# tensorboy/centerpose

Measured on AMD Instinct MI355X. Metric: images/sec end-to-end (backbone+decode), DLA-34 512x512, higher is better.
Workload: dtype f32

## Files before the change

### centerpose_amd/csrc/head_wino24.hip

```cpp
#include "igemm.h"

#define HW_THREADS 512
#define HW_PH 18
#define HW_PW 18
#define HW_PWP 20
#define HW_C 64
#define HW_CGS (HW_C / 4)
#define HW_CG (HW_PH * HW_PWP * 4)
#define HW_PATCH (HW_CGS * HW_CG)
#define HW_F4 (HW_PH * HW_PW * HW_CGS)
#define HW_SLOTS ((HW_F4 + HW_THREADS - 1) / HW_THREADS)
#define HW_LDR 36
#define HW_RED (16 * 32 * HW_LDR)
#define HW_LDM 36
#define HW_MID (256 * HW_LDM)
#define HW_SMEM_FLOATS (2 * HW_RED)
#define HW_SMEM_FLOATS_MM (HW_RED + HW_MID > HW_PATCH ? HW_RED + HW_MID : HW_PATCH)

typedef float hw_v2 __attribute__((ext_vector_type(2)));
typedef float hw_v4 __attribute__((ext_vector_type(4)));

struct HwHead {
    const float* w2;
    const float* b2;
    float* out2;
    int n2, ld2, act2;
};
struct HwGrid {
    int tilesX, tilesY;
    unsigned mTx, mTy;
};
__device__ __forceinline__ hw_v4 hw_lds4(const float* p) { return *reinterpret_cast<const hw_v4*>(p); }
__device__ __forceinline__ int hw_div(int n, int d, unsigned magic) { return d == 1 ? n : (int)__umulhi((unsigned)n, magic); }

template <int N2, int MM>
__global__ __launch_bounds__(HW_THREADS, 1) void head_wino24_kernel(const ConvArgs a, const HwGrid gd, const HwHead hd)
{
    extern __shared__ __attribute__((aligned(16))) float smem[];
    const int tid = threadIdx.x, lane = tid & 63, wv = __builtin_amdgcn_readfirstlane(tid >> 6);
    const int xi = wv & 3, vh = wv >> 2;
    const int h = lane >> 5, m = lane & 31;
    const int NTILES = (a.Cout + 31) >> 5;
    int t_ = ig_xcd_remap(blockIdx.x, gridDim.x), q_;
    q_ = hw_div(t_, gd.tilesX, gd.mTx); const int tx = t_ - q_ * gd.tilesX; t_ = q_;
    q_ = hw_div(t_, gd.tilesY, gd.mTy); const int ty = t_ - q_ * gd.tilesY;
    const int b = q_;
    const int y0 = ty * 16, x0 = tx * 16;
    const int ld = a.srcLd[0];
    const float* __restrict__ x = a.src[0];

    {
        float4 rg[HW_SLOTS];
        int lo[HW_SLOTS];
        bool ok[HW_SLOTS];
#pragma unroll
        for (int s = 0; s < HW_SLOTS; ++s) {
            const int idx = tid + s * HW_THREADS;
            const int pp = idx / HW_CGS, q = idx % HW_CGS;
            const int py = pp / HW_PW, px = pp - py * HW_PW;
            const int gy = y0 - 1 + py, gx = x0 - 1 + px;
            const bool inl = idx < HW_F4;
            ok[s] = inl && gy >= 0 && gy < a.H && gx >= 0 && gx < a.W;
            const int go = ok[s] ? ((b * a.H + gy) * a.W + gx) * ld + q * 4 : 0;
            lo[s] = inl ? ((q * HW_PH + py) * HW_PWP + (px ^ ((py >> 1) & 3))) * 4 : -1;
            rg[s] = ig_ldg4(x + go);
        }
#pragma unroll
        for (int s = 0; s < HW_SLOTS; ++s)
            if (lo[s] >= 0) {
                float4 v = rg[s];
                if (!ok[s]) v = make_float4(0.f, 0.f, 0.f, 0.f);
                *reinterpret_cast<float4*>(smem + lo[s]) = v;
            }
    }
    const float* up = a.w + ((size_t)xi * NTILES * (HW_C / 8)) * 1536 + (size_t)(3 * vh) * 256 + lane * 4;
    const int nlin = NTILES * (HW_C / 8);
    float4 bq[2][3];
#pragma unroll
    for (int nu = 0; nu < 3; ++nu) bq[0][nu] = ig_ldg4(up + nu * 256);
    __syncthreads();

    const int rA = xi == 0 ? 0 : (xi == 2 ? 2 : 1);
    const int rB = xi == 2 ? 1 : (xi == 3 ? 3 : 2);
    const float sg1 = xi == 1 ? 1.f : -1.f;
    const hw_v2 sg = {sg1, sg1};
    const int tyy = m >> 2, txx = m & 3;
    const int sA = (tyy + (rA >> 1)) & 3, sB = (tyy + (rB >> 1)) & 3;
    const int baseA = ((2 * tyy + rA) * HW_PWP + 4 * txx) * 4 + h * HW_CG;
    const int baseB = ((2 * tyy + rB) * HW_PWP + 4 * txx) * 4 + h * HW_CG;
    int offA[4], offB[4];
#pragma unroll
    for (int jj = 0; jj < 4; ++jj) { offA[jj] = baseA + ((jj ^ sA) << 2); offB[jj] = baseB + ((jj ^ sB) << 2); }
    hw_v2 vl[HW_C / 8][3], vhh[HW_C / 8][3];
#pragma unroll
    for (int kc = 0; kc < HW_C / 8; ++kc) {
        const float* pc = smem + kc * 2 * HW_CG;
        hw_v2 tl[5], th[5];
        if (vh == 0) {
#pragma unroll
            for (int j = 0; j < 5; ++j) {
                const hw_v4 da = hw_lds4(pc + offA[j & 3] + (j >> 2) * 16), db = hw_lds4(pc + offB[j & 3] + (j >> 2) * 16);
                tl[j] = __builtin_elementwise_fma(sg, db.xy, da.xy);
                th[j] = __builtin_elementwise_fma(sg, db.zw, da.zw);
            }
        } else {
#pragma unroll
            for (int j = 0; j < 5; ++j) {
                const int jc = j + 1;
                const hw_v4 da = hw_lds4(pc + offA[jc & 3] + (jc >> 2) * 16), db = hw_lds4(pc + offB[jc & 3] + (jc >> 2) * 16);
                tl[j] = __builtin_elementwise_fma(sg, db.xy, da.xy);
                th[j] = __builtin_elementwise_fma(sg, db.zw, da.zw);
            }
        }
        const hw_v2 k4 = {4.f, 4.f}, kn4 = {-4.f, -4.f}, k2 = {2.f, 2.f}, kn2 = {-2.f, -2.f};
        if (vh == 0) {
            const hw_v2 al = __builtin_elementwise_fma(kn4, tl[2], tl[4]), ah = __builtin_elementwise_fma(kn4, th[2], th[4]);
            const hw_v2 bl = __builtin_elementwise_fma(kn4, tl[1], tl[3]), bh = __builtin_elementwise_fma(kn4, th[1], th[3]);
            vl[kc][0] = __builtin_elementwise_fma(k4, tl[0] - tl[2], tl[4] - tl[2]); vhh[kc][0] = __builtin_elementwise_fma(k4, th[0] - th[2], th[4] - th[2]);
            vl[kc][1] = al + bl; vhh[kc][1] = ah + bh;
            vl[kc][2] = al - bl; vhh[kc][2] = ah - bh;
        } else {
            const hw_v2 cl = tl[3] - tl[1], ch = th[3] - th[1];
            const hw_v2 fl = tl[2] - tl[0], fh = th[2] - th[0];
            vl[kc][0] = __builtin_elementwise_fma(k2, fl, cl); vhh[kc][0] = __builtin_elementwise_fma(k2, fh, ch);
            vl[kc][1] = __builtin_elementwise_fma(kn2, fl, cl); vhh[kc][1] = __builtin_elementwise_fma(kn2, fh, ch);
            vl[kc][2] = __builtin_elementwise_fma(kn4, fl, tl[4] - tl[2]); vhh[kc][2] = __builtin_elementwise_fma(kn4, fh, th[4] - th[2]);
        }
#pragma unroll
        for (int nu = 0; nu < 3; ++nu) asm volatile("" : "+v"(vl[kc][nu]), "+v"(vhh[kc][nu]));
        __builtin_amdgcn_sched_barrier(0);
    }
    __syncthreads();

    float acc2[2][2][N2 > 0 ? N2 : 1];
#pragma unroll
    for (int i = 0; i < 2; ++i)
#pragma unroll
        for (int k = 0; k < 2; ++k)
#pragma unroll
            for (int j = 0; j < (N2 > 0 ? N2 : 1); ++j) acc2[i][k][j] = 0.f;
    f32x16 acc2m;
#pragma unroll
    for (int r = 0; r < 16; ++r) acc2m[r] = 0.f;
    constexpr int J0 = MM ? 32 : 0;
    float* const mid = smem + HW_RED;
    const int n4 = tid & 7, bb = (tid >> 3) & 1, mi = tid >> 4;
    const int ity = mi >> 2, itx = mi & 3;
    const int itrd = (bb * 32 + mi) * HW_LDR + n4 * 4;
    const int wpo = (wv * 64 + m) * HW_LDR + 4 * h;

    int lin = 0;
    if constexpr (!MM) {
        hw_v4 sc = {0.f, 0.f, 0.f, 0.f}, sh = sc, w2r[N2];
#pragma unroll
        for (int j = 0; j < N2; ++j) w2r[j] = sc;
        hw_v4 rq[8];
        auto red_read = [&](int P) __attribute__((always_inline)) {
            int rbase = itrd + P * HW_RED;
            asm volatile("" : "+v"(rbase));
            const float* rp = smem + rbase;
#pragma unroll
            for (int w = 0; w < 8; ++w) rq[w] = hw_lds4(rp + w * 64 * HW_LDR);
        };
        auto red_sum = [&](int P) __attribute__((always_inline)) {
            const hw_v4 r0 = rq[0] + rq[4], r1 = rq[1] + rq[5], r2 = rq[2] + rq[6], r3 = rq[3] + rq[7];
            hw_v4 yv[2];
            yv[0] = (r0 + r1) + r2;
            yv[1] = (r1 - r2) - r3;
#pragma unroll
            for (int aa = 0; aa < 2; ++aa) {
                hw_v4 v = __builtin_elementwise_fma(yv[aa], sc, sh);
                v = (hw_v4){cp_relu(v.x), cp_relu(v.y), cp_relu(v.z), cp_relu(v.w)};
#pragma unroll
                for (int j = 0; j < N2; ++j) {
                    const hw_v4 w = w2r[j];
                    acc2[P][aa][j] = fmaf(v.w, w.w, fmaf(v.z, w.z, fmaf(v.y, w.y, fmaf(v.x, w.x, acc2[P][aa][j]))));
                }
            }
        };
#pragma unroll 1
        for (int nt = 0; nt < NTILES; ++nt) {
            const bool prev = nt > 0;
            f32x16 acc[3];
#pragma unroll
            for (int nu = 0; nu < 3; ++nu)
#pragma unroll
                for (int r = 0; r < 16; ++r) acc[nu][r] = 0.f;
#pragma unroll
            for (int kc = 0; kc < HW_C / 8; ++kc) {
                ++lin;
                const float* un = up + (size_t)(lin < nlin ? lin : nlin - 1) * 1536;
                __builtin_amdgcn_sched_barrier(0);
#pragma unroll
                for (int nu = 0; nu < 3; ++nu) {
                    if (nu == 1) {
#pragma unroll
                        for (int q = 0; q < 3; ++q) bq[(kc + 1) & 1][q] = ig_ldg4(un + q * 256);
                        __builtin_amdgcn_sched_barrier(0);
                    }
                    if (nu == 2 && prev) {
                        if (kc == 0) red_read(0);
                        if (kc == 2) red_sum(0);
                        if (kc == 4) red_read(1);
                        if (kc == 6) red_sum(1);
                        __builtin_amdgcn_sched_barrier(0);
                    }
                    const float4 bbv = bq[kc & 1][nu];
                    acc[nu] = __builtin_amdgcn_mfma_f32_32x32x2f32(bbv.x, vl[kc][nu].x, acc[nu], 0, 0, 0);
                    acc[nu] = __builtin_amdgcn_mfma_f32_32x32x2f32(bbv.y, vl[kc][nu].y, acc[nu], 0, 0, 0);
                    acc[nu] = __builtin_amdgcn_mfma_f32_32x32x2f32(bbv.z, vhh[kc][nu].x, acc[nu], 0, 0, 0);
                    acc[nu] = __builtin_amdgcn_mfma_f32_32x32x2f32(bbv.w, vhh[kc][nu].y, acc[nu], 0, 0, 0);
                }
                __builtin_amdgcn_sched_barrier(0);
            }
            const int ncol = nt * 32 + n4 * 4;
            sc = *reinterpret_cast<const hw_v4*>(a.scale + ncol);
            sh = *reinterpret_cast<const hw_v4*>(a.shift + ncol);
#pragma unroll
            for (int j = 0; j < N2; ++j) w2r[j] = *reinterpret_cast<const hw_v4*>(hd.w2 + (size_t)j * hd.ld2 + ncol);
            if (prev) __syncthreads();
#pragma unroll
            for (int P = 0; P < 2; ++P) {
                int wbase = wpo + P * HW_RED;
                asm volatile("" : "+v"(wbase));
                float* wq = smem + wbase;
#pragma unroll
                for (int j = 0; j < 4; ++j) {
                    hw_v4 q[3];
#pragma unroll
                    for (int nu = 0; nu < 3; ++nu) q[nu] = (hw_v4){acc[nu][4 * j], acc[nu][4 * j + 1], acc[nu][4 * j + 2], acc[nu][4 * j + 3]};
                    hw_v4 c0, c1;
                    if (vh == 0) {
                        const hw_v4 s1 = q[1] + q[2], d1 = q[1] - q[2];
                        c0 = P == 0 ? q[0] + s1 : s1;
                        c1 = d1;
                    } else {
                        const hw_v4 s2 = q[0] + q[1], d2 = q[0] - q[1];
                        c0 = P == 0 ? s2 : 4.f * s2;
                        c1 = P == 0 ? 2.f * d2 : 8.f * d2 + q[2];
                    }
                    *reinterpret_cast<hw_v4*>(wq + 8 * j) = c0;
                    *reinterpret_cast<hw_v4*>(wq + 32 * HW_LDR + 8 * j) = c1;
                }
            }
            __syncthreads();
        }
        red_read(0); red_sum(0);
        red_read(1); red_sum(1);
    } else {
#pragma unroll 1
    for (int nt = 0; nt < NTILES; ++nt) {
        f32x16 acc[3];
#pragma unroll
        for (int nu = 0; nu < 3; ++nu)
#pragma unroll
            for (int r = 0; r < 16; ++r) acc[nu][r] = 0.f;
#pragma unroll
        for (int kc = 0; kc < HW_C / 8; ++kc) {
            ++lin;
            const float* un = up + (size_t)(lin < nlin ? lin : nlin - 1) * 1536;
            __builtin_amdgcn_sched_barrier(0);
#pragma unroll
            for (int nu = 0; nu < 3; ++nu) {
                if (nu == 1) {
#pragma unroll
                    for (int q = 0; q < 3; ++q) bq[(kc + 1) & 1][q] = ig_ldg4(un + q * 256);
                    __builtin_amdgcn_sched_barrier(0);
                }
                const float4 bbv = bq[kc & 1][nu];
                acc[nu] = __builtin_amdgcn_mfma_f32_32x32x2f32(bbv.x, vl[kc][nu].x, acc[nu], 0, 0, 0);
                acc[nu] = __builtin_amdgcn_mfma_f32_32x32x2f32(bbv.y, vl[kc][nu].y, acc[nu], 0, 0, 0);
                acc[nu] = __builtin_amdgcn_mfma_f32_32x32x2f32(bbv.z, vhh[kc][nu].x, acc[nu], 0, 0, 0);
                acc[nu] = __builtin_amdgcn_mfma_f32_32x32x2f32(bbv.w, vhh[kc][nu].y, acc[nu], 0, 0, 0);
            }
            __builtin_amdgcn_sched_barrier(0);
        }

        const int ncol = nt * 32 + n4 * 4;
        const hw_v4 sc = *reinterpret_cast<const hw_v4*>(a.scale + ncol), sh = *reinterpret_cast<const hw_v4*>(a.shift + ncol);
        hw_v4 w2r[N2 > 0 ? N2 : 1];
#pragma unroll
        for (int j = 0; j < N2; ++j) w2r[j] = *reinterpret_cast<const hw_v4*>(hd.w2 + (size_t)(J0 + j) * hd.ld2 + ncol);
        hw_v4 w2f[MM ? 4 : 1];
#pragma unroll
        for (int P = 0; P < 2; ++P) {
            if (MM && P == 1) __syncthreads();
            int wbase = wpo + (MM ? 0 : P * HW_RED), rbase = itrd + (MM ? 0 : P * HW_RED);
            asm volatile("" : "+v"(wbase), "+v"(rbase));
            float* wq = smem + wbase;
#pragma unroll
            for (int j = 0; j < 4; ++j) {
                hw_v4 q[3];
#pragma unroll
                for (int nu = 0; nu < 3; ++nu) q[nu] = (hw_v4){acc[nu][4 * j], acc[nu][4 * j + 1], acc[nu][4 * j + 2], acc[nu][4 * j + 3]};
                hw_v4 c0, c1;
                if (vh == 0) {
                    const hw_v4 s1 = q[1] + q[2], d1 = q[1] - q[2];
                    c0 = P == 0 ? q[0] + s1 : s1;
                    c1 = d1;
                } else {
                    const hw_v4 s2 = q[0] + q[1], d2 = q[0] - q[1];
                    c0 = P == 0 ? s2 : 4.f * s2;
                    c1 = P == 0 ? 2.f * d2 : 8.f * d2 + q[2];
                }
                *reinterpret_cast<hw_v4*>(wq + 8 * j) = c0;
                *reinterpret_cast<hw_v4*>(wq + 32 * HW_LDR + 8 * j) = c1;
            }
            if constexpr (MM) {
                if (P == 1) {
                    const int nmm = hd.n2 < 32 ? hd.n2 : 32;
                    const bool live = m < nmm;
                    const float* wrow = hd.w2 + (size_t)(live ? m : nmm - 1) * hd.ld2 + nt * 32 + 4 * h;
#pragma unroll
                    for (int s4 = 0; s4 < 4; ++s4) {
                        const float4 t4 = ig_ldg4(wrow + 8 * s4);
                        w2f[s4] = live ? (hw_v4){t4.x, t4.y, t4.z, t4.w} : (hw_v4){0.f, 0.f, 0.f, 0.f};
                    }
                }
            }
            __syncthreads();
            const float* rp = smem + rbase;
            hw_v4 r0 = hw_lds4(rp) + hw_lds4(rp + 4 * 64 * HW_LDR);
            const hw_v4 r1 = hw_lds4(rp + 64 * HW_LDR) + hw_lds4(rp + 5 * 64 * HW_LDR);
            const hw_v4 r2 = hw_lds4(rp + 2 * 64 * HW_LDR) + hw_lds4(rp + 6 * 64 * HW_LDR);
            const hw_v4 r3 = hw_lds4(rp + 3 * 64 * HW_LDR) + hw_lds4(rp + 7 * 64 * HW_LDR);
            hw_v4 yv[2];
            yv[0] = (r0 + r1) + r2;
            yv[1] = (r1 - r2) - r3;
#pragma unroll
            for (int aa = 0; aa < 2; ++aa) {
                hw_v4 v = __builtin_elementwise_fma(yv[aa], sc, sh);
                v = (hw_v4){cp_relu(v.x), cp_relu(v.y), cp_relu(v.z), cp_relu(v.w)};
#pragma unroll
                for (int j = 0; j < N2; ++j) {
                    const hw_v4 w = w2r[j];
                    acc2[P][aa][j] = fmaf(v.w, w.w, fmaf(v.z, w.z, fmaf(v.y, w.y, fmaf(v.x, w.x, acc2[P][aa][j]))));
                }
                if constexpr (MM) {
                    *reinterpret_cast<hw_v4*>(mid + ((2 * ity + aa) * 16 + 4 * itx + 2 * P + bb) * HW_LDM + n4 * 4) = v;
                }
            }
        }
        if constexpr (MM) {
            __syncthreads();
            const float* mp = mid + (32 * wv + m) * HW_LDM + 4 * h;
            hw_v4 mf[4];
#pragma unroll
            for (int s4 = 0; s4 < 4; ++s4) mf[s4] = hw_lds4(mp + 8 * s4);
#pragma unroll
            for (int s4 = 0; s4 < 4; ++s4) {
                acc2m = __builtin_amdgcn_mfma_f32_32x32x2f32(w2f[s4].x, mf[s4].x, acc2m, 0, 0, 0);
                acc2m = __builtin_amdgcn_mfma_f32_32x32x2f32(w2f[s4].y, mf[s4].y, acc2m, 0, 0, 0);
                acc2m = __builtin_amdgcn_mfma_f32_32x32x2f32(w2f[s4].z, mf[s4].z, acc2m, 0, 0, 0);
                acc2m = __builtin_amdgcn_mfma_f32_32x32x2f32(w2f[s4].w, mf[s4].w, acc2m, 0, 0, 0);
            }
            __syncthreads();
        }
    }

    }
    const size_t HW = (size_t)a.H * a.W;
    if constexpr (MM) {
        const int p = 32 * wv + m, ox = x0 + (p & 15), oy = y0 + (p >> 4);
        const int nmm = hd.n2 < 32 ? hd.n2 : 32;
        if (ox < a.W && oy < a.H) {
#pragma unroll
            for (int r = 0; r < 16; ++r) {
                const int j = (r & 3) + 8 * (r >> 2) + 4 * h;
                if (j < nmm) hd.out2[((size_t)b * hd.n2 + j) * HW + (size_t)oy * a.W + ox] = cp_act(acc2m[r] + hd.b2[j], hd.act2);
            }
        }
    }
    if constexpr (N2 > 0) {
#pragma unroll
        for (int P = 0; P < 2; ++P) {
            const int ox = x0 + 4 * itx + 2 * P + bb, oy = y0 + 2 * ity;
#pragma unroll
            for (int aa = 0; aa < 2; ++aa)
#pragma unroll
                for (int j = 0; j < N2; ++j) {
                    float v = acc2[P][aa][j];
                    v += __shfl_xor(v, 1);
                    v += __shfl_xor(v, 2);
                    v += __shfl_xor(v, 4);
                    if ((tid & 7) == 0 && J0 + j < hd.n2 && ox < a.W && oy + aa < a.H)
                        hd.out2[((size_t)b * hd.n2 + J0 + j) * HW + (size_t)(oy + aa) * a.W + ox] = cp_act(v + hd.b2[J0 + j], hd.act2);
                }
        }
    }
}

static unsigned hw_magic(int d) { return d <= 1 ? 0u : (unsigned)(((1ull << 32) + (unsigned)d - 1) / (unsigned)d); }

template <int N2, int MM>
static int launch_head_wino24(const ConvArgs& a, hipStream_t s, const HwHead& hd)
{
    const int smem = (MM ? HW_SMEM_FLOATS_MM : HW_SMEM_FLOATS) * 4;
    static CpLdsGuard guard;
    {
        const hipError_t e = guard.ensure((const void*)head_wino24_kernel<N2, MM>, smem);
        if (e != hipSuccess) { cp_set_error("head_wino24: cannot reserve %d B LDS: %s", smem, hipGetErrorString(e)); return 2; }
    }
    HwGrid gd;
    gd.tilesX = cp_cdiv(a.W, 16); gd.tilesY = cp_cdiv(a.H, 16);
    gd.mTx = hw_magic(gd.tilesX); gd.mTy = hw_magic(gd.tilesY);
    const long long grid = (long long)a.B * gd.tilesX * gd.tilesY;
    const long long dmax = gd.tilesX > gd.tilesY ? gd.tilesX : gd.tilesY;
    if (grid * dmax >= (1ll << 32)) { cp_set_error("head_wino24: grid %lld too large", grid); return 1; }
    hipLaunchKernelGGL((head_wino24_kernel<N2, MM>), dim3((unsigned)grid), dim3(HW_THREADS), smem, s, a, gd, hd);
    cp_note_kernel("head_wino24_kernel<%d, %d>", N2, MM);
    return 0;
}

int cp_launch_head3x3_1x1_w24(const ConvArgs& a, const float* w2, const float* b2, float* out2, int n2, int ld2, int act2, hipStream_t s)
{
    const bool ok = a.nsrc == 1 && a.kh == 3 && a.kw == 3 && a.sy == 1 && a.sx == 1 && a.py == 1 && a.px == 1 && a.Ho == a.H &&
                    a.Wo == a.W && a.srcC[0] == 64 && a.srcLd[0] % 4 == 0 && a.Cout % 32 == 0 && a.act == CP_ACT_RELU && !a.res &&
                    n2 >= 1 && n2 <= 34 && ld2 % 4 == 0 && ld2 >= a.Cout &&
                    (((size_t)a.src[0] | (size_t)a.w | (size_t)w2 | (size_t)a.scale | (size_t)a.shift) & 15) == 0 &&
                    (long long)a.B * a.H * a.W * a.srcLd[0] < (1ll << 31);
    if (!ok) return -1;
    HwHead hd;
    hd.w2 = w2; hd.b2 = b2; hd.out2 = out2; hd.n2 = n2; hd.ld2 = ld2; hd.act2 = act2;
    if (n2 == 1) return launch_head_wino24<1, 0>(a, s, hd);
    if (n2 == 2) return launch_head_wino24<2, 0>(a, s, hd);
    if (n2 <= 32) return launch_head_wino24<0, 1>(a, s, hd);
    if (n2 == 33) return launch_head_wino24<1, 1>(a, s, hd);
    return launch_head_wino24<2, 1>(a, s, hd);
}
```

### centerpose_amd/ops.py

```python
import ctypes
import os

import torch

from . import _lib

ACT_NONE, ACT_RELU, ACT_SIGMOID, ACT_HSWISH, ACT_HSIGMOID = 0, 1, 2, 3, 4
BN_EPS = 1e-5


class ConvDesc(ctypes.Structure):
    _fields_ = [(n, ctypes.c_int) for n in ("nsrc",)] + [("srcC", ctypes.c_int * 4), ("srcLd", ctypes.c_int * 4)] + \
        [(n, ctypes.c_int) for n in ("B", "H", "W", "Ho", "Wo", "kh", "kw", "sy", "sx", "py", "px", "K", "ldw", "Cout",
                                     "resLd", "outLd", "outNCHW", "OH", "OW", "osy", "osx", "ooy", "oox", "act",
                                     "inNCHW", "tile", "nsub", "ksplit")]


class DcnDesc(ctypes.Structure):
    _fields_ = [(n, ctypes.c_int) for n in ("B", "H", "W", "C", "srcLd", "Ho", "Wo", "kh", "kw", "sy", "sx", "py", "px",
                                            "dily", "dilx", "K", "ldw", "Cout", "omLd", "omSigmoid", "outLd",
                                            "outNCHW", "act", "tile", "ksplit", "dg")]


def round_up(x, m):
# ... 150 lines not shown
        t.stride(0) == t.shape[1] * t.stride(1), "NHWC tensor with dense pixels expected"
    return t.stride(2)


BATCH_INVARIANT = os.environ.get("CP_BATCH_INVARIANT", "0") == "1"


def rule_batch(B):
    return 1 if BATCH_INVARIANT else B


SPLIT_BF16 = os.environ.get("CP_SPLIT_BF16", "0") == "1"
SPLIT_BF16_TILES = ((128, 128), (128, 64), (64, 128), (64, 64))


def split_bf16_weight(wp, ldw):
    L = _lib.lib()
    rows, K = wp.shape
    assert rows % ldw == 0 and K % 16 == 0 and wp.is_contiguous()
    L.cp_split_bf16_weight_floats.restype = ctypes.c_size_t
    wb = torch.empty((L.cp_split_bf16_weight_floats(rows, K),), dtype=torch.float32, device=wp.device)
    _lib.check(L.cp_split_bf16_weights_f32(_lib.ptr(wp), rows, ldw, K, _lib.ptr(wb), _lib.stream()), "cp_split_bf16_weights_f32")
    return wb


def split_bf16_tile(M, ldw, nsub=1, ksplit=1, force=False, K=None):
    if ldw % 64:
        return None
    code = lambda bm, bn: 3000000 + bm * 1000 + bn
    forced = os.environ.get("CP_SPLIT_BF16_TILE")
    if forced:
        bm, bn = (int(v) for v in forced.split("x")) if "x" in forced else (128, int(forced))
        return code(bm, bn if ldw % bn == 0 else 64)
    blocks = lambda bm, bn: ((M + bm - 1) // bm) * max(1, nsub) * max(1, ksplit) * (ldw // bn)
    floor = 0 if force else int(os.environ.get("CP_SPLIT_BF16_MINBLOCKS", "512"))
    if floor == 0:
        return code(128, 128) if ldw % 128 == 0 and blocks(128, 128) >= 256 else code(128, 64)
    if ksplit > 1:
        return None
    order = ((64, 64),) if K is not None and K <= 64 else ((128, 128), (64, 128), (64, 64))
    for bm, bn in order:
        if ldw % bn == 0 and blocks(bm, bn) >= floor:
            return code(bm, bn)
    return None


def conv2d(srcs, wp, scale, shift, out, **kw):
    conv2d_launch(srcs, wp, scale, shift, out, **kw).run()
    return out


def conv2d_launch(srcs, wp, scale, shift, out, *, kh, kw, stride=1, pad=0, cout, act=ACT_NONE, res=None, out_nchw=False,
                  in_nchw=False, Ho=None, Wo=None, pad_yx=None, out_scatter=None, tile=0, wino=None, nsub=1, ksplit=0, split_bf16=None):
    d = ConvDesc()
    d.nsrc = len(srcs)
    if in_nchw:
        x = srcs[0]
        B, C, H, W = x.shape
        d.srcC[0], d.srcLd[0] = C, 0
        assert x.is_contiguous()
    else:
        B, H, W, _ = srcs[0].shape
        for i, s in enumerate(srcs):
            assert s.shape[:3] == srcs[0].shape[:3]
            d.srcC[i], d.srcLd[i] = s.shape[3], _ld(s)
    py, px = pad_yx if pad_yx is not None else (pad, pad)
    if Ho is None:
        Ho = (H + 2 * py - kh) // stride + 1
        Wo = (W + 2 * px - kw) // stride + 1
    d.B, d.H, d.W, d.Ho, d.Wo = B, H, W, Ho, Wo
    d.kh, d.kw, d.sy, d.sx, d.py, d.px = kh, kw, stride, stride, py, px
    assert wp.shape[0] % nsub == 0
    d.K, d.ldw, d.Cout, d.nsub = wp.shape[1], wp.shape[0] // nsub, cout, nsub
    d.resLd = _ld(res) if res is not None else 0
    d.outNCHW = 1 if out_nchw else 0
    d.ksplit = ksplit
    if ksplit > 1:
        assert res is None and act == ACT_NONE and not out_nchw and out.is_contiguous() and (wino is not None or (len(srcs) == 1 and not in_nchw and nsub == 1))
        assert tuple(out.shape[:2]) == (ksplit, B * Ho * Wo) and out.shape[2] >= cout and out.shape[2] % 4 == 0
        d.OH, d.OW, d.outLd = Ho, Wo, out.shape[2]
    elif out_nchw:
        d.OH, d.OW, d.outLd = out.shape[2], out.shape[3], 0
        assert out.is_contiguous() and out.shape[1] == cout
    else:
        d.OH, d.OW, d.outLd = out.shape[1], out.shape[2], _ld(out)
    d.osy, d.osx, d.ooy, d.oox = out_scatter if out_scatter is not None else (1, 1, 0, 0)
    d.act, d.inNCHW, d.tile = act, 1 if in_nchw else 0, tile
    for t in (wp, scale, shift, wino):
        assert t is None or t.is_contiguous()
    if wino is not None:
        assert len(srcs) == 1 and not in_nchw
        return Launch("cp_conv3x3_winograd_f32", d, [srcs[0], wino, scale, shift, res, out])
    if (SPLIT_BF16 if split_bf16 is None else split_bf16) and tile == 0 and not in_nchw:
        code = split_bf16_tile(rule_batch(B) * Ho * Wo, d.ldw, nsub, ksplit, force=split_bf16 is True, K=d.K)
        c16 = kh == 3 and kw == 3 and len(srcs) == 1 and srcs[0].shape[3] == 16 and cout <= 32
        if code is not None and not c16 and all(s.data_ptr() % 16 == 0 for s in srcs):
            d.tile = code
            wp = split_bf16_weight(wp, d.ldw)
    return Launch("cp_conv2d_f32", d, list(srcs) + [None] * (4 - len(srcs)) + [wp, scale, shift, res, out])


ConvDesc4 = ConvDesc * 4


def conv3x3_group_launch(members, whole):
    assert 1 <= len(members) <= 4
    members = sorted(members, key=lambda mm: -mm["x"].shape[3])
    d = ConvDesc4()
    cols = [[None] * 4 for _ in range(6)]
    for i, mm in enumerate(members):
        one = conv2d_launch([mm["x"]], mm["wp"], mm["scale"], mm["shift"], mm["out"], kh=3, kw=3, stride=1, pad=1, cout=mm["cout"],
                            act=mm["act"], res=mm["res"], wino=mm["u24"], tile=WINO24)
        ctypes.memmove(ctypes.addressof(d[i]), ctypes.addressof(one.desc), ctypes.sizeof(ConvDesc))
        for k, t in enumerate((mm["x"], mm["u24"], mm["scale"], mm["shift"], mm["res"], mm["out"])):
            cols[k][i] = t
            assert t is None or k in (0, 4, 5) or t.is_contiguous()
        assert mm["out"].untyped_storage().data_ptr() == whole.untyped_storage().data_ptr()
    return Launch("cp_conv3x3_winograd24_group_f32", d, [t for col in cols for t in col] + [whole], [len(members)])


ConvDesc8 = ConvDesc * 8
GROUP_MAX = 8


def conv2d_group_launch(members, whole):
    assert 1 <= len(members) <= GROUP_MAX
    members = sorted(members, key=lambda mm: -mm["wp"].shape[1])
    d = ConvDesc8()
    cols = [[None] * GROUP_MAX for _ in range(6)]
    for i, mm in enumerate(members):
        assert mm["wp"].shape[0] % 64 == 0
        one = conv2d_launch([mm["x"]], mm["wp"], mm["scale"], mm["shift"], mm["out"], kh=mm["k"], kw=mm["k"], stride=mm["stride"],
                            pad=mm["pad"], cout=mm["cout"], act=mm["act"], res=mm.get("res"), split_bf16=False)
        ctypes.memmove(ctypes.addressof(d[i]), ctypes.addressof(one.desc), ctypes.sizeof(ConvDesc))
        for k, t in enumerate((mm["x"], mm["wp"], mm["scale"], mm["shift"], mm.get("res"), mm["out"])):
            cols[k][i] = t
            assert t is None or k in (0, 4, 5) or t.is_contiguous()
        assert mm["out"].untyped_storage().data_ptr() == whole.untyped_storage().data_ptr()
    return Launch("cp_conv2d_group_f32", d, [t for col in cols for t in col] + [whole], [len(members)])


def head3x3_1x1_eligible(x, hc, n2):
    B, H, W, C = x.shape
    B = rule_batch(B)
    return C == 64 and hc % 32 == 0 and hc >= 128 and 1 <= n2 <= 34 and B * ((H + 7) // 8) * ((W + 15) // 16) >= 512


def head_wino24_wanted(x, n2):
    B, H, W, _ = x.shape
    B = rule_batch(B)
    mode = os.environ.get("CP_HEAD24", "1")
    if mode == "0" or B * ((H + 15) // 16) * ((W + 15) // 16) < 256:
        return False
    return mode == "all" or n2 <= 32


def head3x3_1x1_launch(x, u, scale, shift, w2, b2, out2, *, hc, act2=ACT_NONE, wino24=False):
    B, H, W, C = x.shape
    n2, ld2 = w2.shape
    assert out2.is_contiguous() and tuple(out2.shape) == (B, n2, H, W) and w2.is_contiguous() and b2.numel() >= n2
    d = ConvDesc()
    d.nsrc = 1
    d.srcC[0], d.srcLd[0] = C, _ld(x)
    d.B, d.H, d.W, d.Ho, d.Wo = B, H, W, H, W
    d.kh, d.kw, d.sy, d.sx, d.py, d.px = 3, 3, 1, 1, 1, 1
    d.K, d.ldw, d.Cout = 9 * C, round_up(hc, 64), hc
    d.resLd, d.outLd, d.outNCHW = 0, hc, 0
    d.OH, d.OW, d.osy, d.osx, d.ooy, d.oox = H, W, 1, 1, 0, 0
    d.act, d.inNCHW, d.tile, d.nsub = ACT_RELU, 0, WINO24 if wino24 else 0, 1
    return Launch("cp_head3x3_1x1_f32", d, [x, u, scale, shift, w2, b2, out2], [n2, ld2, act2])


def wino_eligible(cin, k, stride, pad, nsrc=1):
    return k == 3 and stride == 1 and pad == 1 and nsrc == 1 and cin % 16 == 0 and cin >= 32


def pack_wino_weight(wp, cin, cout):
    L = _lib.lib()
    assert wp.shape[1] == 9 * cin and wp.shape[0] >= cout and wp.is_contiguous()
    L.cp_winograd_weight_floats.restype = ctypes.c_size_t
    n = L.cp_winograd_weight_floats(cin, cout)
    assert n > 0, "winograd: C must be a multiple of 16"
    u = torch.empty((n,), dtype=torch.float32, device=wp.device)
    _lib.check(L.cp_winograd_pack_f32(_lib.ptr(wp), _lib.ptr(u), cin, cout, _lib.stream()), "cp_winograd_pack_f32")
    return u


def pack_wino24_weight(wp, cin, cout):
    L = _lib.lib()
    assert wp.shape[1] == 9 * cin and wp.shape[0] >= cout and wp.is_contiguous()
    L.cp_winograd24_weight_floats.restype = ctypes.c_size_t
    n = L.cp_winograd24_weight_floats(cin, cout)
    assert n > 0, "winograd: C must be a multiple of 16"
    u = torch.empty((n,), dtype=torch.float32, device=wp.device)
    _lib.check(L.cp_winograd24_pack_f32(_lib.ptr(wp), _lib.ptr(u), cin, cout, _lib.stream()), "cp_winograd24_pack_f32")
    return u


WINO24 = 24


def wino24_wanted(B, H, W, cin, cout):
    if os.environ.get("CP_WINO24", "1") == "0" or cin % 16 or cin < 32:
        return False
    minc, mincout, minblocks = (int(v) for v in os.environ.get("CP_WINO24_RULE", "32,16,256").split(","))
    blocks = rule_batch(B) * ((H + 15) // 16) * ((W + 15) // 16) * ((cout + 31) // 32)
    return cin >= minc and cout >= mincout and blocks >= minblocks


def dcn_v2(x, om, wp, scale, shift, out, **kw):
    dcn_v2_launch(x, om, wp, scale, shift, out, **kw).run()
    return out


def _pair(v):
    return (int(v[0]), int(v[1])) if isinstance(v, (tuple, list)) else (int(v), int(v))


def dcn_v2_launch(x, om, wp, scale, shift, out, *, cout, kh=3, kw=3, stride=1, pad=1, dil=1, om_sigmoid=True,
                  act=ACT_NONE, out_nchw=False, tile=0, ksplit=0, dg=1):
    B, H, W, C = x.shape
    d = DcnDesc()
    (sy, sx), (py, px), (dy, dx) = _pair(stride), _pair(pad), _pair(dil)
    Ho = (H + 2 * py - (dy * (kh - 1) + 1)) // sy + 1
    Wo = (W + 2 * px - (dx * (kw - 1) + 1)) // sx + 1
    assert om.shape[:3] == (B, Ho, Wo)
    d.B, d.H, d.W, d.C, d.srcLd, d.Ho, d.Wo = B, H, W, C, _ld(x), Ho, Wo
    d.kh, d.kw, d.sy, d.sx, d.py, d.px, d.dily, d.dilx = kh, kw, sy, sx, py, px, dy, dx
    d.K, d.ldw, d.Cout = wp.shape[1], wp.shape[0], cout
    d.omLd, d.omSigmoid = _ld(om), 1 if om_sigmoid else 0
    d.outNCHW = 1 if out_nchw else 0
    d.act, d.tile, d.ksplit, d.dg = act, tile, ksplit, dg
    if ksplit > 1:
        assert tuple(out.shape) == (ksplit, B * Ho * Wo, wp.shape[0]) and out.is_contiguous() and cout == wp.shape[0] and act == ACT_NONE
        d.outLd = wp.shape[0]
    else:
        d.outLd = 0 if out_nchw else _ld(out)
    return Launch("cp_dcn_v2_f32", d, [x, om, wp, scale, shift, out])


def wino_ksplit(B, H, W, cin, cout):
    blocks = rule_batch(B) * ((H + 7) // 8) * ((W + 15) // 16) * ((cout + 31) // 32)
    stages = cin // 16
    S = 1
    while blocks * S < 512 and stages // (2 * S) >= 4:
        S *= 2
    return S if blocks < 256 else 1


def conv_ksplit(M, ldw, K):
    if ldw % 64 != 0:
        return 1
    blocks = ((M + 63) // 64) * (ldw // 64)
    if blocks >= 400:
        return 1
    for S in (2, 3, 4):
        if blocks * S >= 512 and (K // 16) // S >= 16:
            return S
    return 1


def dcn_ksplit(M, ldw, taps=9):
    if ldw % 64 != 0 or taps < 3:
        return 1
    blocks = -(-M // 64) * (ldw // 64)
    return 3 if blocks < 512 else 1


def splitk_reduce_launch(ws, scale, shift, out, *, cout, act=ACT_NONE):
    S, M, ldw = ws.shape
    assert ws.is_contiguous() and out.shape[0] * out.shape[1] * out.shape[2] == M and scale.numel() >= ldw and shift.numel() >= ldw
    return Launch("cp_splitk_reduce_f32", None, [ws, scale, shift, out], [S, M, ldw, act, _ld(out), cout])


def maxpool2d_launch(x, out, k, s, p):
    B, H, W, C = x.shape
    return Launch("cp_maxpool2d_nhwc_f32", None, [x, out], [_ld(x), _ld(out), B, H, W, C, k, s, p])


def maxpool2d(x, out, k, s, p):
    maxpool2d_launch(x, out, k, s, p).run()
    return out


def pack_dw_deconv_weight(w):
    C, _, k, _ = w.shape
    return w.reshape(C, k * k).t().contiguous().float()


def dw_deconv_add_launch(x, wk, add, out, f):
    B, H, W, C = x.shape
    assert wk.is_contiguous()
    return Launch("cp_dw_deconv_add_nhwc_f32", None, [x, wk, add, out],
                  [_ld(x), _ld(add) if add is not None else 0, _ld(out), B, H, W, C, f])


def dw_deconv_add(x, wk, add, out, f):
    dw_deconv_add_launch(x, wk, add, out, f).run()
    return out


def pack_dw_weight(w):
    C, _, k, _ = w.shape
    return w.reshape(C, k * k).t().contiguous().float()


def dwconv2d_launch(x, wk, scale, shift, out, k, stride, pad, act=ACT_NONE):
# ... 166 lines not shown
```

Measured before the change: 2232.

## Pipeline MM-variant Winograd head epilogue into next tile's MFMA loop

Measured after the change: 2244 (median of 6 runs). Within noise of the previous version (+0.5%).

```diff
diff --git a/centerpose_amd/csrc/head_wino24.hip b/centerpose_amd/csrc/head_wino24.hip
--- a/centerpose_amd/csrc/head_wino24.hip
+++ b/centerpose_amd/csrc/head_wino24.hip
@@ -12,10 +12,7 @@
 #define HW_SLOTS ((HW_F4 + HW_THREADS - 1) / HW_THREADS)
 #define HW_LDR 36
 #define HW_RED (16 * 32 * HW_LDR)
-#define HW_LDM 36
-#define HW_MID (256 * HW_LDM)
 #define HW_SMEM_FLOATS (2 * HW_RED)
-#define HW_SMEM_FLOATS_MM (HW_RED + HW_MID > HW_PATCH ? HW_RED + HW_MID : HW_PATCH)
 
 typedef float hw_v2 __attribute__((ext_vector_type(2)));
 typedef float hw_v4 __attribute__((ext_vector_type(4)));
@@ -143,61 +140,98 @@
 #pragma unroll
     for (int r = 0; r < 16; ++r) acc2m[r] = 0.f;
     constexpr int J0 = MM ? 32 : 0;
-    float* const mid = smem + HW_RED;
     const int n4 = tid & 7, bb = (tid >> 3) & 1, mi = tid >> 4;
     const int ity = mi >> 2, itx = mi & 3;
     const int itrd = (bb * 32 + mi) * HW_LDR + n4 * 4;
     const int wpo = (wv * 64 + m) * HW_LDR + 4 * h;
 
+    hw_v4 sc = {0.f, 0.f, 0.f, 0.f}, sh = sc, w2r[N2 > 0 ? N2 : 1];
+#pragma unroll
+    for (int j = 0; j < (N2 > 0 ? N2 : 1); ++j) w2r[j] = sc;
+    hw_v4 rq[8];
+    auto red_read = [&](int P) __attribute__((always_inline)) {
+        int rbase = itrd + P * HW_RED;
+        asm volatile("" : "+v"(rbase));
+        const float* rp = smem + rbase;
+#pragma unroll
+        for (int w = 0; w < 8; ++w) rq[w] = hw_lds4(rp + w * 64 * HW_LDR);
+    };
+    auto red_sum = [&](int P) __attribute__((always_inline)) {
+        const hw_v4 r0 = rq[0] + rq[4], r1 = rq[1] + rq[5], r2 = rq[2] + rq[6], r3 = rq[3] + rq[7];
+        hw_v4 yv[2];
+        yv[0] = (r0 + r1) + r2;
+        yv[1] = (r1 - r2) - r3;
+#pragma unroll
+        for (int aa = 0; aa < 2; ++aa) {
+            hw_v4 v = __builtin_elementwise_fma(yv[aa], sc, sh);
+            v = (hw_v4){cp_relu(v.x), cp_relu(v.y), cp_relu(v.z), cp_relu(v.w)};
+#pragma unroll
+            for (int j = 0; j < N2; ++j) {
+                const hw_v4 w = w2r[j];
+                acc2[P][aa][j] = fmaf(v.w, w.w, fmaf(v.z, w.z, fmaf(v.y, w.y, fmaf(v.x, w.x, acc2[P][aa][j]))));
+            }
+        }
+    };
+    const int cw = wv & 3, aw = wv >> 2;
+    int mrd = (cw >> 1) * HW_RED + (aw * 64 + (cw & 1) * 32 + m) * HW_LDR + 4 * h;
+    if constexpr (MM) asm volatile("" : "+v"(mrd));
+    const float sgm1 = aw ? -1.f : 1.f;
+    const int nmm = hd.n2 < 32 ? hd.n2 : 32;
+    const int w2mo = (m < nmm ? m : nmm - 1) * hd.ld2 + 4 * h;
+    float4 w2f = make_float4(0.f, 0.f, 0.f, 0.f);
+    auto mm_load = [&](int q, int tile) __attribute__((always_inline)) {
+        const int ncol = tile * 32 + 8 * q + 4 * h;
+        sc = *reinterpret_cast<const hw_v4*>(a.scale + ncol);
+        sh = *reinterpret_cast<const hw_v4*>(a.shift + ncol);
+        w2f = ig_ldg4(hd.w2 + (w2mo + tile * 32 + 8 * q));
+#pragma unroll
+        for (int j = 0; j < N2; ++j) w2r[j] = *reinterpret_cast<const hw_v4*>(hd.w2 + (size_t)(J0 + j) * hd.ld2 + ncol);
+    };
+    auto mm_read = [&](int q) __attribute__((always_inline)) {
+        const float* rp = smem + mrd + 8 * q;
+#pragma unroll
+        for (int w = 0; w < 3; ++w) { rq[w] = hw_lds4(rp + w * 64 * HW_LDR); rq[3 + w] = hw_lds4(rp + (4 + w) * 64 * HW_LDR); }
+    };
+    auto mm_sum = [&]() __attribute__((always_inline)) {
+        const hw_v4 t0 = rq[0] + rq[3], t1 = rq[1] + rq[4], t2 = rq[2] + rq[5];
+        const hw_v4 y = {fmaf(sgm1, t2.x, fmaf(sgm1, t1.x, t0.x)), fmaf(sgm1, t2.y, fmaf(sgm1, t1.y, t0.y)),
+                         fmaf(sgm1, t2.z, fmaf(sgm1, t1.z, t0.z)), fmaf(sgm1, t2.w, fmaf(sgm1, t1.w, t0.w))};
+        hw_v4 v = __builtin_elementwise_fma(y, sc, sh);
+        v = __builtin_elementwise_max(v, (hw_v4){0.f, 0.f, 0.f, 0.f});
+#pragma unroll
+        for (int j = 0; j < N2; ++j) {
+            const hw_v4 w = w2r[j];
+            acc2[0][0][j] = fmaf(v.w, w.w, fmaf(v.z, w.z, fmaf(v.y, w.y, fmaf(v.x, w.x, acc2[0][0][j]))));
+        }
+        acc2m = __builtin_amdgcn_mfma_f32_32x32x2f32(w2f.x, v.x, acc2m, 0, 0, 0);
+        acc2m = __builtin_amdgcn_mfma_f32_32x32x2f32(w2f.y, v.y, acc2m, 0, 0, 0);
+        acc2m = __builtin_amdgcn_mfma_f32_32x32x2f32(w2f.z, v.z, acc2m, 0, 0, 0);
+        acc2m = __builtin_amdgcn_mfma_f32_32x32x2f32(w2f.w, v.w, acc2m, 0, 0, 0);
+    };
+
     int lin = 0;
-    if constexpr (!MM) {
-        hw_v4 sc = {0.f, 0.f, 0.f, 0.f}, sh = sc, w2r[N2];
-#pragma unroll
-        for (int j = 0; j < N2; ++j) w2r[j] = sc;
-        hw_v4 rq[8];
-        auto red_read = [&](int P) __attribute__((always_inline)) {
-            int rbase = itrd + P * HW_RED;
-            asm volatile("" : "+v"(rbase));
-            const float* rp = smem + rbase;
-#pragma unroll
-            for (int w = 0; w < 8; ++w) rq[w] = hw_lds4(rp + w * 64 * HW_LDR);
-        };
-        auto red_sum = [&](int P) __attribute__((always_inline)) {
-            const hw_v4 r0 = rq[0] + rq[4], r1 = rq[1] + rq[5], r2 = rq[2] + rq[6], r3 = rq[3] + rq[7];
-            hw_v4 yv[2];
-            yv[0] = (r0 + r1) + r2;
-            yv[1] = (r1 - r2) - r3;
-#pragma unroll
-            for (int aa = 0; aa < 2; ++aa) {
-                hw_v4 v = __builtin_elementwise_fma(yv[aa], sc, sh);
-                v = (hw_v4){cp_relu(v.x), cp_relu(v.y), cp_relu(v.z), cp_relu(v.w)};
-#pragma unroll
-                for (int j = 0; j < N2; ++j) {
-                    const hw_v4 w = w2r[j];
-                    acc2[P][aa][j] = fmaf(v.w, w.w, fmaf(v.z, w.z, fmaf(v.y, w.y, fmaf(v.x, w.x, acc2[P][aa][j]))));
+#pragma unroll 1
+    for (int nt = 0; nt < NTILES; ++nt) {
+        const bool prev = nt > 0;
+        const int ntp = prev ? nt - 1 : 0;
+        f32x16 acc[3];
+#pragma unroll
+        for (int nu = 0; nu < 3; ++nu)
+#pragma unroll
+            for (int r = 0; r < 16; ++r) acc[nu][r] = 0.f;
+#pragma unroll
+        for (int kc = 0; kc < HW_C / 8; ++kc) {
+            ++lin;
+            const float* un = up + (size_t)(lin < nlin ? lin : nlin - 1) * 1536;
+            __builtin_amdgcn_sched_barrier(0);
+#pragma unroll
+            for (int nu = 0; nu < 3; ++nu) {
+                if (nu == 1) {
+#pragma unroll
+                    for (int q = 0; q < 3; ++q) bq[(kc + 1) & 1][q] = ig_ldg4(un + q * 256);
+                    __builtin_amdgcn_sched_barrier(0);
                 }
-            }
-        };
-#pragma unroll 1
-        for (int nt = 0; nt < NTILES; ++nt) {
-            const bool prev = nt > 0;
-            f32x16 acc[3];
-#pragma unroll
-            for (int nu = 0; nu < 3; ++nu)
-#pragma unroll
-                for (int r = 0; r < 16; ++r) acc[nu][r] = 0.f;
-#pragma unroll
-            for (int kc = 0; kc < HW_C / 8; ++kc) {
-                ++lin;
-                const float* un = up + (size_t)(lin < nlin ? lin : nlin - 1) * 1536;
-                __builtin_amdgcn_sched_barrier(0);
-#pragma unroll
-                for (int nu = 0; nu < 3; ++nu) {
-                    if (nu == 1) {
-#pragma unroll
-                        for (int q = 0; q < 3; ++q) bq[(kc + 1) & 1][q] = ig_ldg4(un + q * 256);
-                        __builtin_amdgcn_sched_barrier(0);
-                    }
+                if constexpr (!MM) {
                     if (nu == 2 && prev) {
                         if (kc == 0) red_read(0);
                         if (kc == 2) red_sum(0);
@@ -205,67 +239,15 @@
                         if (kc == 6) red_sum(1);
                         __builtin_amdgcn_sched_barrier(0);
                     }
-                    const float4 bbv = bq[kc & 1][nu];
-                    acc[nu] = __builtin_amdgcn_mfma_f32_32x32x2f32(bbv.x, vl[kc][nu].x, acc[nu], 0, 0, 0);
-                    acc[nu] = __builtin_amdgcn_mfma_f32_32x32x2f32(bbv.y, vl[kc][nu].y, acc[nu], 0, 0, 0);
-                    acc[nu] = __builtin_amdgcn_mfma_f32_32x32x2f32(bbv.z, vhh[kc][nu].x, acc[nu], 0, 0, 0);
-                    acc[nu] = __builtin_amdgcn_mfma_f32_32x32x2f32(bbv.w, vhh[kc][nu].y, acc[nu], 0, 0, 0);
-                }
-                __builtin_amdgcn_sched_barrier(0);
-            }
-            const int ncol = nt * 32 + n4 * 4;
-            sc = *reinterpret_cast<const hw_v4*>(a.scale + ncol);
-            sh = *reinterpret_cast<const hw_v4*>(a.shift + ncol);
-#pragma unroll
-            for (int j = 0; j < N2; ++j) w2r[j] = *reinterpret_cast<const hw_v4*>(hd.w2 + (size_t)j * hd.ld2 + ncol);
-            if (prev) __syncthreads();
-#pragma unroll
-            for (int P = 0; P < 2; ++P) {
-                int wbase = wpo + P * HW_RED;
-                asm volatile("" : "+v"(wbase));
-                float* wq = smem + wbase;
-#pragma unroll
-                for (int j = 0; j < 4; ++j) {
-                    hw_v4 q[3];
-#pragma unroll
-                    for (int nu = 0; nu < 3; ++nu) q[nu] = (hw_v4){acc[nu][4 * j], acc[nu][4 * j + 1], acc[nu][4 * j + 2], acc[nu][4 * j + 3]};
-                    hw_v4 c0, c1;
-                    if (vh == 0) {
-                        const hw_v4 s1 = q[1] + q[2], d1 = q[1] - q[2];
-                        c0 = P == 0 ? q[0] + s1 : s1;
-                        c1 = d1;
-                    } else {
-                        const hw_v4 s2 = q[0] + q[1], d2 = q[0] - q[1];
-                        c0 = P == 0 ? s2 : 4.f * s2;
-                        c1 = P == 0 ? 2.f * d2 : 8.f * d2 + q[2];
+                } else {
+                    if (nu == 2) {
+                        if ((kc & 1) == 0) mm_load(kc >> 1, ntp);
+                        if (prev) {
+                            if ((kc & 1) == 0) mm_read(kc >> 1);
+                            else mm_sum();
+                        }
+                        __builtin_amdgcn_sched_barrier(0);
                     }
-                    *reinterpret_cast<hw_v4*>(wq + 8 * j) = c0;
-                    *reinterpret_cast<hw_v4*>(wq + 32 * HW_LDR + 8 * j) = c1;
-                }
-            }
-            __syncthreads();
-        }
-        red_read(0); red_sum(0);
-        red_read(1); red_sum(1);
-    } else {
-#pragma unroll 1
-    for (int nt = 0; nt < NTILES; ++nt) {
-        f32x16 acc[3];
-#pragma unroll
-        for (int nu = 0; nu < 3; ++nu)
-#pragma unroll
-            for (int r = 0; r < 16; ++r) acc[nu][r] = 0.f;
-#pragma unroll
-        for (int kc = 0; kc < HW_C / 8; ++kc) {
-            ++lin;
-            const float* un = up + (size_t)(lin < nlin ? lin : nlin - 1) * 1536;
-            __builtin_amdgcn_sched_barrier(0);
-#pragma unroll
-            for (int nu = 0; nu < 3; ++nu) {
-                if (nu == 1) {
-#pragma unroll
-                    for (int q = 0; q < 3; ++q) bq[(kc + 1) & 1][q] = ig_ldg4(un + q * 256);
-                    __builtin_amdgcn_sched_barrier(0);
                 }
                 const float4 bbv = bq[kc & 1][nu];
                 acc[nu] = __builtin_amdgcn_mfma_f32_32x32x2f32(bbv.x, vl[kc][nu].x, acc[nu], 0, 0, 0);
@@ -275,18 +257,18 @@
             }
             __builtin_amdgcn_sched_barrier(0);
         }
-
-        const int ncol = nt * 32 + n4 * 4;
-        const hw_v4 sc = *reinterpret_cast<const hw_v4*>(a.scale + ncol), sh = *reinterpret_cast<const hw_v4*>(a.shift + ncol);
-        hw_v4 w2r[N2 > 0 ? N2 : 1];
-#pragma unroll
-        for (int j = 0; j < N2; ++j) w2r[j] = *reinterpret_cast<const hw_v4*>(hd.w2 + (size_t)(J0 + j) * hd.ld2 + ncol);
-        hw_v4 w2f[MM ? 4 : 1];
+        if constexpr (!MM) {
+            const int ncol = nt * 32 + n4 * 4;
+            sc = *reinterpret_cast<const hw_v4*>(a.scale + ncol);
+            sh = *reinterpret_cast<const hw_v4*>(a.shift + ncol);
+#pragma unroll
+            for (int j = 0; j < N2; ++j) w2r[j] = *reinterpret_cast<const hw_v4*>(hd.w2 + (size_t)j * hd.ld2 + ncol);
+        }
+        if (prev) __syncthreads();
 #pragma unroll
         for (int P = 0; P < 2; ++P) {
-            if (MM && P == 1) __syncthreads();
-            int wbase = wpo + (MM ? 0 : P * HW_RED), rbase = itrd + (MM ? 0 : P * HW_RED);
-            asm volatile("" : "+v"(wbase), "+v"(rbase));
+            int wbase = wpo + P * HW_RED;
+            asm volatile("" : "+v"(wbase));
             float* wq = smem + wbase;
 #pragma unroll
             for (int j = 0; j < 4; ++j) {
@@ -306,72 +288,38 @@
                 *reinterpret_cast<hw_v4*>(wq + 8 * j) = c0;
                 *reinterpret_cast<hw_v4*>(wq + 32 * HW_LDR + 8 * j) = c1;
             }
-            if constexpr (MM) {
-                if (P == 1) {
-                    const int nmm = hd.n2 < 32 ? hd.n2 : 32;
-                    const bool live = m < nmm;
-                    const float* wrow = hd.w2 + (size_t)(live ? m : nmm - 1) * hd.ld2 + nt * 32 + 4 * h;
-#pragma unroll
-                    for (int s4 = 0; s4 < 4; ++s4) {
-                        const float4 t4 = ig_ldg4(wrow + 8 * s4);
-                        w2f[s4] = live ? (hw_v4){t4.x, t4.y, t4.z, t4.w} : (hw_v4){0.f, 0.f, 0.f, 0.f};
-                    }
-                }
-            }
-            __syncthreads();
-            const float* rp = smem + rbase;
-            hw_v4 r0 = hw_lds4(rp) + hw_lds4(rp + 4 * 64 * HW_LDR);
-            const hw_v4 r1 = hw_lds4(rp + 64 * HW_LDR) + hw_lds4(rp + 5 * 64 * HW_LDR);
-            const hw_v4 r2 = hw_lds4(rp + 2 * 64 * HW_LDR) + hw_lds4(rp + 6 * 64 * HW_LDR);
-            const hw_v4 r3 = hw_lds4(rp + 3 * 64 * HW_LDR) + hw_lds4(rp + 7 * 64 * HW_LDR);
-            hw_v4 yv[2];
-            yv[0] = (r0 + r1) + r2;
-            yv[1] = (r1 - r2) - r3;
-#pragma unroll
-            for (int aa = 0; aa < 2; ++aa) {
-                hw_v4 v = __builtin_elementwise_fma(yv[aa], sc, sh);
-                v = (hw_v4){cp_relu(v.x), cp_relu(v.y), cp_relu(v.z), cp_relu(v.w)};
-#pragma unroll
-                for (int j = 0; j < N2; ++j) {
-                    const hw_v4 w = w2r[j];
-                    acc2[P][aa][j] = fmaf(v.w, w.w, fmaf(v.z, w.z, fmaf(v.y, w.y, fmaf(v.x, w.x, acc2[P][aa][j]))));
-                }
-                if constexpr (MM) {
-                    *reinterpret_cast<hw_v4*>(mid + ((2 * ity + aa) * 16 + 4 * itx + 2 * P + bb) * HW_LDM + n4 * 4) = v;
-                }
-            }
-        }
-        if constexpr (MM) {
-            __syncthreads();
-            const float* mp = mid + (32 * wv + m) * HW_LDM + 4 * h;
-            hw_v4 mf[4];
-#pragma unroll
-            for (int s4 = 0; s4 < 4; ++s4) mf[s4] = hw_lds4(mp + 8 * s4);
-#pragma unroll
-            for (int s4 = 0; s4 < 4; ++s4) {
-                acc2m = __builtin_amdgcn_mfma_f32_32x32x2f32(w2f[s4].x, mf[s4].x, acc2m, 0, 0, 0);
-                acc2m = __builtin_amdgcn_mfma_f32_32x32x2f32(w2f[s4].y, mf[s4].y, acc2m, 0, 0, 0);
-                acc2m = __builtin_amdgcn_mfma_f32_32x32x2f32(w2f[s4].z, mf[s4].z, acc2m, 0, 0, 0);
-                acc2m = __builtin_amdgcn_mfma_f32_32x32x2f32(w2f[s4].w, mf[s4].w, acc2m, 0, 0, 0);
-            }
-            __syncthreads();
-        }
-    }
-
+        }
+        __syncthreads();
+    }
+    if constexpr (!MM) {
+        red_read(0); red_sum(0);
+        red_read(1); red_sum(1);
+    } else {
+#pragma unroll
+        for (int q = 0; q < 4; ++q) { mm_load(q, NTILES - 1); mm_read(q); mm_sum(); }
     }
     const size_t HW = (size_t)a.H * a.W;
     if constexpr (MM) {
-        const int p = 32 * wv + m, ox = x0 + (p & 15), oy = y0 + (p >> 4);
-        const int nmm = hd.n2 < 32 ? hd.n2 : 32;
+        const int le = __lane_id(), me = le & 31, he = le >> 5;
+        const int ox = x0 + 4 * (me & 3) + cw, oy = y0 + 2 * (me >> 2) + aw;
         if (ox < a.W && oy < a.H) {
 #pragma unroll
             for (int r = 0; r < 16; ++r) {
-                const int j = (r & 3) + 8 * (r >> 2) + 4 * h;
+                const int j = (r & 3) + 8 * (r >> 2) + 4 * he;
                 if (j < nmm) hd.out2[((size_t)b * hd.n2 + j) * HW + (size_t)oy * a.W + ox] = cp_act(acc2m[r] + hd.b2[j], hd.act2);
             }
         }
-    }
-    if constexpr (N2 > 0) {
+        if constexpr (N2 > 0) {
+#pragma unroll
+            for (int j = 0; j < N2; ++j) {
+                float v = acc2[0][0][j];
+                v += __shfl_xor(v, 32);
+                if (he == 0 && J0 + j < hd.n2 && ox < a.W && oy < a.H)
+                    hd.out2[((size_t)b * hd.n2 + J0 + j) * HW + (size_t)oy * a.W + ox] = cp_act(v + hd.b2[J0 + j], hd.act2);
+            }
+        }
+    }
+    if constexpr (N2 > 0 && !MM) {
 #pragma unroll
         for (int P = 0; P < 2; ++P) {
             const int ox = x0 + 4 * itx + 2 * P + bb, oy = y0 + 2 * ity;
@@ -395,7 +343,7 @@
 template <int N2, int MM>
 static int launch_head_wino24(const ConvArgs& a, hipStream_t s, const HwHead& hd)
 {
-    const int smem = (MM ? HW_SMEM_FLOATS_MM : HW_SMEM_FLOATS) * 4;
+    const int smem = HW_SMEM_FLOATS * 4;
     static CpLdsGuard guard;
     {
         const hipError_t e = guard.ensure((const void*)head_wino24_kernel<N2, MM>, smem);
diff --git a/centerpose_amd/ops.py b/centerpose_amd/ops.py
--- a/centerpose_amd/ops.py
+++ b/centerpose_amd/ops.py
@@ -326,7 +326,7 @@
     mode = os.environ.get("CP_HEAD24", "1")
     if mode == "0" or B * ((H + 15) // 16) * ((W + 15) // 16) < 256:
         return False
-    return mode == "all" or n2 <= 32
+    return mode == "all" or n2 <= 34
 
 
 def head3x3_1x1_launch(x, u, scale, shift, w2, b2, out2, *, hc, act2=ACT_NONE, wino24=False):
```
